# fallenshock/SinDDM

Hardware: AMD Instinct MI355X
Metric: diffusion steps/sec (finest scale) + imgs/sec full multi-scale sample, 1/2/4/8 GPU (higher is better)
Workload: dtype f32 (3x3 convs: binary16 hi/lo split products -- Winograd-domain GEMMs with all 4 MFMA terms, fp32 accumulate; fp32-equivalent, error vs float64 = the fp32 oracle's: tests/test_gpu_h2.py; everything else fp32); 1 GPU; C3: 6-scale pyramid, T=1000, finest scale 411x512, batch 64 per GPU, dim=160; batch_per_gpu=64, global_batch=64, scale=5, parallelism=independent chains over 1 GPU(s), one all-gather of the images

## Files before the change

### sinddm_amd/csrc/conv_args.h

```cpp
#pragma once
#include "common.h"

namespace sinddm {

struct ConvArgs {
    const float* in;
    const float* in2;
    const float* resid;
    const float* aux;
    const float* w3;
    const float* w1;
    const float* bias;
    const float* zero;
    float* out;
    float* out_pre;
    int B, H, W, Cin, Cin2, Cout;
    int nch3, nch1;
    int tilesX, tilesY, ntiles, tiles_per_xcd;
    int coblks;
    int mtp;
    int act;
    const float* wsinv;
    const float* amax_in;
    float* amax_out;
    int Wt;
};

template <int NT, int WV = 4>
struct ConvGeom {
    static constexpr int TW = 32;
    static constexpr int TPR = TW / 16;
    static constexpr int RPW = NT / TPR;
    static constexpr int TH = WV * RPW;
    static constexpr int RS = TW + 2;
    static constexpr int HR = TH + 2;
    static constexpr int PS = ((HR * RS - 16 + 31) / 32) * 32 + 16;
    static constexpr int IN_ELEMS = KC * HR * RS;
    static constexpr int IREGS = (IN_ELEMS + CONV_THREADS - 1) / CONV_THREADS;
};

template <int MT, int NT, int WV = 4>
struct ConvCfg {
    using G = ConvGeom<NT, WV>;
    static constexpr int CO_LDS = (MT * 16) % 32 == 16 ? MT * 16 : MT * 16 + 16;
    static constexpr int W3_F4 = 9 * KC * CO_LDS / 4;
    static constexpr int W1_F4 = KC * CO_LDS / 4;
    static constexpr int WREGS = (W3_F4 + CONV_THREADS - 1) / CONV_THREADS;
    static constexpr int LDS_FLOATS = 9 * KC * CO_LDS + KC * G::PS;
};

struct ConvProfiler {
    bool on = false;
    int used = 0;
    double flops = 0.0;
    double exec_flops = 0.0;
    static constexpr int MAXREC = 8192;
    hipEvent_t ev[2 * MAXREC];
    int created = 0;
    unsigned char kind[MAXREC];
    unsigned char gen[MAXREC];
    double rec_flops[MAXREC], rec_exec[MAXREC];
    void note(int k, double fl, double ex, int g = 0) {
        kind[used] = (unsigned char)k; gen[used] = (unsigned char)g; rec_flops[used] = fl; rec_exec[used] = ex;
        flops += fl; exec_flops += ex; ++used;
    }
    bool begin(hipStream_t st) {
        if (!on || used >= MAXREC) return false;
        while (created <= used) {
            (void)hipEventCreate(&ev[2 * created]);
            (void)hipEventCreate(&ev[2 * created + 1]);
            ++created;
        }
        (void)hipEventRecord(ev[2 * used], st);
        return true;
    }
    void end(hipStream_t st, int k, double fl, double ex, int g = 0) {
        (void)hipEventRecord(ev[2 * used + 1], st);
        note(k, fl, ex, g);
    }
};
ConvProfiler& conv_profiler();

}
```

### sinddm_amd/csrc/conv_wh.h

```cpp
#pragma once
#include <utility>
#include "split16.h"

namespace sinddm {

template <class F, int... I>
__device__ __forceinline__ void wh_static_for_impl(F&& f, std::integer_sequence<int, I...>) {
    (f(std::integral_constant<int, I>{}), ...);
}
template <int N, class F>
__device__ __forceinline__ void wh_static_for(F&& f) {
    wh_static_for_impl(f, std::make_integer_sequence<int, N>{});
}

#ifndef WH_ABL
#define WH_ABL 0
#endif
#ifndef WH_MIXLO
#define WH_MIXLO 1
#endif
#ifndef WH_NT
#define WH_NT 6
#endif
#ifdef WH_TIMING
__device__ unsigned long long g_wh_seg[8 * 256 * 8 * 32];
#define WH_SEG(slot) do { if (j == 2) g_wh_seg[((p.mtp * 256 + blockIdx.x) * 8 + wv) * 32 + (slot)] = __builtin_amdgcn_s_memtime(); } while (0)
#else
#define WH_SEG(slot) do {} while (0)
#endif
constexpr int WH_TH = 8, WH_TW = 32;
constexpr int WH_RS = 40;
constexpr int WH_PS = 408;
constexpr int WH_RAW = 16 * WH_PS * 4;
constexpr int WH_V = 24 * 2 * 64 * 16;
constexpr int WH_XS = 36;
constexpr int WH_X = 2 * 6 * 32 * WH_XS * 4;
constexpr int WH_LDS = 160 * 1024;
constexpr int WH_REGION = WH_LDS - WH_RAW;
constexpr int WH_VB = WH_REGION - WH_V;
static_assert(WH_X <= WH_VB && WH_V + WH_X <= WH_REGION && WH_VB % 16 == 0, "exchange buffer beside either V buffer");
constexpr int WH_TARGET_EXP = 10;
constexpr int WH_COB = 80;

inline bool wh_shape_ok(int cin, int cout) { return cin >= 32 && cin % 16 == 0 && cout % WH_COB == 0; }
inline long long wh_image_halfs(int cin, int cout) { return (long long)(cout / WH_COB) * (cin / 16) * 24 * 5 * 512; }

__device__ __forceinline__ int wh_shift_for(float m, int target) {
    const unsigned bits = __float_as_uint(m) & 0x7fffffffu;
    const int e = (int)(bits >> 23);
    if (e == 0 || e == 255) return 0;
    int s = target - (e - 127);
    return s > 100 ? 100 : (s < -100 ? -100 : s);
}

__device__ __forceinline__ void wh_u24(const float* __restrict__ w, long long base, int transpose, double (&u)[24]) {
    const double G2[4][3] = {{1., 0., 0.}, {.5, .5, .5}, {.5, -.5, .5}, {0., 0., 1.}};
    const double G4[6][3] = {{1. / 4, 0., 0.}, {-1. / 6, -1. / 6, -1. / 6}, {-1. / 6, 1. / 6, -1. / 6},
                             {1. / 24, 1. / 12, 1. / 6}, {1. / 24, -1. / 12, 1. / 6}, {0., 0., 1.}};
    double g[3][3];
#pragma unroll
    for (int a = 0; a < 3; ++a)
#pragma unroll
        for (int b = 0; b < 3; ++b) g[a][b] = (double)(transpose ? w[base + (2 - a) * 3 + (2 - b)] : w[base + a * 3 + b]);
#pragma unroll
    for (int i = 0; i < 4; ++i)
#pragma unroll
        for (int j = 0; j < 6; ++j) {
            double acc = 0.;
#pragma unroll
            for (int a = 0; a < 3; ++a) {
                double r = 0.;
#pragma unroll
                for (int b = 0; b < 3; ++b) r += G4[j][b] * g[a][b];
                acc += G2[i][a] * r;
            }
            u[i * 6 + j] = acc;
        }
}

__global__ __launch_bounds__(256) void wh_wscale_kernel(const float* __restrict__ w, float* __restrict__ wsinv, int cin,
                                                         int cout, int transpose) {
    const int m = blockIdx.x;
    const int M = transpose ? cin : cout, K = transpose ? cout : cin;
    float mx = 0.f;
    if (m < M)
        for (int k = threadIdx.x; k < K; k += 256) {
            double u[24];
            wh_u24(w, transpose ? ((long long)k * cin + m) * 9 : ((long long)m * cin + k) * 9, transpose, u);
#pragma unroll
            for (int f = 0; f < 24; ++f) mx = fmaxf(mx, fabsf((float)u[f]));
        }
    __shared__ float red[4];
#pragma unroll
    for (int o = 32; o > 0; o >>= 1) mx = fmaxf(mx, __shfl_xor(mx, o));
    if ((threadIdx.x & 63) == 0) red[threadIdx.x >> 6] = mx;
    __syncthreads();
    if (threadIdx.x == 0 && m < M) {
        mx = fmaxf(fmaxf(red[0], red[1]), fmaxf(red[2], red[3]));
        wsinv[m] = h2_pow2(-h2_shift_for(mx));
    }
}

__global__ __launch_bounds__(256) void wh_pack_kernel(const float* __restrict__ w, const float* __restrict__ wsinv,
                                                       _Float16* __restrict__ img, int cin, int cout, int transpose,
                                                       long long total) {
    const long long i = (long long)blockIdx.x * 256 + threadIdx.x;
    if (i >= total) return;
    const int M = transpose ? cin : cout, K = transpose ? cout : cin;
    const int nch = K / 16;
    long long r = i;
    const int e = (int)(r % 8); r /= 8;
    const int co16 = (int)(r % 16); r /= 16;
    const int kh = (int)(r % 2); r /= 2;
    const int n = (int)(r % 5); r /= 5;
    const int ch = (int)(r % nch); r /= nch;
    const int cb = (int)r;
    const int m = cb * WH_COB + n * 16 + co16;
    const int k = ch * 16 + kh * 8 + e;
    double u[24];
    if (m < M && k < K) wh_u24(w, transpose ? ((long long)k * cin + m) * 9 : ((long long)m * cin + k) * 9, transpose, u);
    else {
#pragma unroll
        for (int f = 0; f < 24; ++f) u[f] = 0.;
    }
    const double sc = m < M ? 1.0 / (double)wsinv[m] : 1.0;
#pragma unroll
    for (int f = 0; f < 24; ++f) {
        const double s = u[f] * sc;
        const _Float16 hi = (_Float16)(float)s;
        const _Float16 lo = (_Float16)(float)(s - (double)(float)hi);
        const long long o = ((((long long)(cb * nch + ch) * 24 + f) * 5 + n) * 2) * 256 + (kh * 16 + co16) * 8 + e;
        img[o] = hi;
        img[o + 256] = lo;
    }
}

inline int wh_pack_launch(const float* w, float* wsinv, void* img, int cin, int cout, int transpose, hipStream_t st) {
    const int M = transpose ? cin : cout, K = transpose ? cout : cin;
    hipLaunchKernelGGL(wh_wscale_kernel, dim3(M), dim3(256), 0, st, w, wsinv, cin, cout, transpose);
    SINDDM_LAUNCH_CHECK();
    const long long total = (long long)(M / WH_COB) * (K / 16) * 5 * 2 * 16 * 8;
    hipLaunchKernelGGL(wh_pack_kernel, dim3((unsigned)((total + 255) / 256)), dim3(256), 0, st, w, wsinv,
                       static_cast<_Float16*>(img), cin, cout, transpose, total);
    SINDDM_LAUNCH_CHECK();
    return 0;
}

__device__ __forceinline__ void wh_barrier() { asm volatile("s_waitcnt lgkmcnt(0)\n\ts_barrier" ::: "memory"); }

__device__ __forceinline__ float wh_dpp_shr2(float old, float src) {
    return __builtin_bit_cast(float, __builtin_amdgcn_update_dpp(__builtin_bit_cast(int, old), __builtin_bit_cast(int, src), 0x112, 0xf, 0xf, false));
}
__device__ __forceinline__ float wh_dpp_shl2(float old, float src) {
    return __builtin_bit_cast(float, __builtin_amdgcn_update_dpp(__builtin_bit_cast(int, old), __builtin_bit_cast(int, src), 0x102, 0xf, 0xf, false));
}

__global__ __launch_bounds__(512) void conv_wh_kernel(ConvArgs p, int items_per_xcd, int wg_per_xcd) {
    typedef __attribute__((address_space(3))) float lds_f;
    extern __shared__ __attribute__((aligned(16))) float smem[];
    unsigned char* const sbytes = reinterpret_cast<unsigned char*>(smem);
    unsigned char* const sRaw = sbytes;
    unsigned char* const sV = sbytes + WH_RAW;
    const unsigned lds0 = (unsigned)(size_t)(lds_f*)smem;

    const int tid = threadIdx.x;
    const int lane = tid & 63;
    const int wv = __builtin_amdgcn_readfirstlane(tid >> 6);
    const int l16 = lane & 15, kq = lane >> 4;
    const int H = p.H, W = p.W;
    const int HW = H * W;
    const int Wt = p.Wt > 0 ? p.Wt : W;
    const int nch = p.nch3;
    const bool big_out = __builtin_amdgcn_readfirstlane((size_t)p.B * p.Cout * HW > ((size_t)1 << 28)) != 0;
    constexpr int OOB = 0x40000000;
    const bool service_rt = wv >= 6;
    const int sv = wv - 6;

    const int t_q = lane & 1, t_tc = (lane >> 1) & 7, t_mg = (lane >> 4) & 1, t_trl = lane >> 5;
    const int t_tr = t_mg * 2 + t_trl, t_t16 = t_trl * 8 + t_tc;
    const int t_rdB = (((sv & 1) * 8 + 4 * t_q) * WH_PS + 2 * t_tr * WH_RS + 4 * t_tc + 4) * 4;
    const int t_rdE = (((sv & 1) * 8 + 4 * t_q) * WH_PS + 2 * t_tr * WH_RS + (t_tc == 7 ? 36 : 3)) * 4;
    const int t_wr0 = ((t_mg * 64 + (sv & 1) * 16 + t_t16) * 16) + t_q * 8;
    const int fj = service_rt ? 0 : wv;
    const int a_rd = ((kq & 1) * 16 + l16) * 16;

    const int xcd = blockIdx.x & 7, ls = blockIdx.x >> 3;
    const int tpi = p.tilesX * p.tilesY;
    struct Item { int b, y0, x0, cb; bool ok; };
    auto decode = [&](int j) {
        Item it;
        const int li = ls + j * wg_per_xcd;
        const int tl = li / p.coblks;
        it.cb = li - tl * p.coblks;
        const int tile = xcd * p.tiles_per_xcd + tl;
        it.ok = li < items_per_xcd && tile < p.ntiles;
        const int tcl = it.ok ? tile : 0;
        it.b = tcl / tpi;
        const int trm = tcl - it.b * tpi;
        const int tyi = trm / p.tilesX;
        it.y0 = tyi * WH_TH;
        it.x0 = (trm - tyi * p.tilesX) * WH_TW;
        return it;
    };
    auto stage_offsets = [&](const Item& it, int (&vo)[2]) {
#pragma unroll
        for (int ps = 0; ps < 2; ++ps) {
            const int qd = ps * 64 + lane;
            const int r = qd / 10, g = qd - r * 10;
            const int gy = it.y0 - 1 + r, gx = it.x0 - 4 + 4 * g;
            vo[ps] = (qd < 100 && gy >= 0 && gy < H && gx >= 0 && gx < W) ? (gy * W + gx) * 4 : OOB;
        }
    };
    auto role_body = [&](auto ROLE) {
    constexpr bool service = decltype(ROLE)::value;
    f32x4 stg[16];
    auto stage_load = [&](const __amdgpu_buffer_rsrc_t& rs, const int (&vo)[2], int c) {
#pragma unroll
        for (int k = 0; k < 8; ++k) {
            const int so = (c * 16 + (sv & 1) * 8 + k) * HW * 4;
            stg[2 * k] = (WH_ABL & 1) ? f32x4{0.f, 0.f, 0.f, 0.f} : __builtin_bit_cast(f32x4, __builtin_amdgcn_raw_buffer_load_b128(rs, vo[0], so, (WH_NT & 1) ? 2 : 0));
            stg[2 * k + 1] = (WH_ABL & 1) ? f32x4{0.f, 0.f, 0.f, 0.f} : __builtin_bit_cast(f32x4, __builtin_amdgcn_raw_buffer_load_b128(rs, vo[1], so, (WH_NT & 1) ? 2 : 0));
        }
    };
    auto stage_write = [&](unsigned char* raw) {
        unsigned char* dst = raw + (sv & 1) * 8 * WH_PS * 4 + lane * 16;
#pragma unroll
        for (int k = 0; k < 8; ++k) {
            *reinterpret_cast<f32x4*>(dst + k * WH_PS * 4) = stg[2 * k];
            if (lane < 36) *reinterpret_cast<f32x4*>(dst + k * WH_PS * 4 + 1024) = stg[2 * k + 1];
        }
    };
    auto in_rsrc = [&](int b) {
        return __builtin_amdgcn_make_buffer_rsrc(const_cast<float*>(p.in + (size_t)b * p.Cin * HW), 0, p.Cin * HW * 4, 0x00020000);
    };

    Item cur = decode(0);
    if (!cur.ok) return;
    int svoff[2] = {OOB, OOB};
#ifndef WH_SVC_PRIO
#define WH_SVC_PRIO 2
#endif
    if constexpr (service) __builtin_amdgcn_s_setprio(WH_SVC_PRIO);
    if constexpr (service) {
        stage_offsets(cur, svoff);
        stage_load(in_rsrc(cur.b), svoff, 0);
    }
    auto item_scale = [&](const Item& it, float& sxo, float& inv) {
        const int xs = p.amax_in ? wh_shift_for(p.amax_in[(size_t)it.b * AMAX_STRIDE], WH_TARGET_EXP) : 0;
        const float sg = (((it.x0 >> 5) + (it.y0 >> 3) + it.b) & 1) ? -1.0f : 1.0f;
        sxo = sg * h2_pow2(xs);
        inv = sg * h2_pow2(-xs);
    };
    int g = 0;
    auto vbuf = [&](int k) { return sV + ((k & 1) ? WH_VB : 0); };
    for (int j = 0;; ++j) {
        const Item nxt = decode(j + 1);
        const int cb = cur.cb, b = cur.b, y0 = cur.y0, x0 = cur.x0;
        float sx, inv_sx;
        item_scale(cur, sx, inv_sx);

        const __amdgpu_buffer_rsrc_t rsin = in_rsrc(b);

        auto transform = [&](const unsigned char* raw, unsigned char* vb, float sxv) {
            if (WH_ABL & 2) return;
            const f32x2 sx2{sxv, sxv};
            const unsigned char* rpB = raw + t_rdB;
            const unsigned char* rpE = raw + t_rdE;
            unsigned char* wp = vb + t_wr0;
            f32x2 d[2][4][6];
#pragma unroll
            for (int pr = 0; pr < 2; ++pr)
#pragma unroll
                for (int rr = 0; rr < 4; ++rr) {
                    const int o = ((2 * pr) * WH_PS + rr * WH_RS) * 4;
                    const f32x4 a4 = *reinterpret_cast<const f32x4*>(rpB + o), b4 = *reinterpret_cast<const f32x4*>(rpB + o + WH_PS * 4);
                    const float ae = *reinterpret_cast<const float*>(rpE + o), be = *reinterpret_cast<const float*>(rpE + o + WH_PS * 4);
                    d[pr][rr][0] = f32x2{wh_dpp_shr2(ae, a4[3]), wh_dpp_shr2(be, b4[3])};
                    d[pr][rr][1] = f32x2{a4[0], b4[0]}; d[pr][rr][2] = f32x2{a4[1], b4[1]};
                    d[pr][rr][3] = f32x2{a4[2], b4[2]}; d[pr][rr][4] = f32x2{a4[3], b4[3]};
                    d[pr][rr][5] = f32x2{wh_dpp_shl2(ae, a4[0]), wh_dpp_shl2(be, b4[0])};
                }
            wh_static_for<4>([&](auto II) {
                constexpr int i = decltype(II)::value;
                h16x2 hi[2][6], lo[2][6];
#pragma unroll
                for (int pr = 0; pr < 2; ++pr) {
                    f32x2 r[6];
#pragma unroll
                    for (int c = 0; c < 6; ++c)
                        r[c] = i == 0 ? d[pr][0][c] - d[pr][2][c] : i == 1 ? d[pr][1][c] + d[pr][2][c]
                             : i == 2 ? d[pr][2][c] - d[pr][1][c] : d[pr][1][c] - d[pr][3][c];
                    const f32x2 s24 = r[4] - 4.f * r[2], s13 = r[3] - 4.f * r[1];
                    const f32x2 u24 = r[4] - r[2], d31 = r[3] - r[1];
                    f32x2 v[6];
                    v[0] = 4.f * r[0] + (r[4] - 5.f * r[2]);
                    v[1] = s24 + s13;
                    v[2] = s24 - s13;
                    v[3] = u24 + 2.f * d31;
                    v[4] = u24 - 2.f * d31;
                    v[5] = 4.f * r[1] + (r[5] - 5.f * r[3]);
#pragma unroll
                    for (int j = 0; j < 6; ++j) {
                        const f32x2 sc = v[j] * sx2;
                        hi[pr][j] = __builtin_convertvector(sc, h16x2);
#if WH_MIXLO
                        lo[pr][j] = h16x2{(_Float16)__builtin_fmaf(v[j].x, sxv, -(float)hi[pr][j].x), (_Float16)__builtin_fmaf(v[j].y, sxv, -(float)hi[pr][j].y)};
#else
                        const f32x2 rem{__builtin_fmaf(v[j].x, sxv, -(float)hi[pr][j].x), __builtin_fmaf(v[j].y, sxv, -(float)hi[pr][j].y)};
                        lo[pr][j] = __builtin_convertvector(rem, h16x2);
#endif
                    }
                }
#pragma unroll
                for (int j = 0; j < 6; ++j) {
                    using h16x4 = __attribute__((ext_vector_type(4))) _Float16;
                    *reinterpret_cast<h16x4*>(wp + (i * 6 + j) * 2048) = h16x4{hi[0][j][0], hi[0][j][1], hi[1][j][0], hi[1][j][1]};
                    *reinterpret_cast<h16x4*>(wp + (i * 6 + j) * 2048 + 512) = h16x4{lo[0][j][0], lo[0][j][1], lo[1][j][0], lo[1][j][1]};
                }
            });
        };

        f32x4 acc[4][2][5];
#pragma unroll
        for (int a = 0; a < 4; ++a)
#pragma unroll
            for (int g = 0; g < 2; ++g)
#pragma unroll
                for (int n = 0; n < 5; ++n) acc[a][g][n] = f32x4{0.f, 0.f, 0.f, 0.f};
        const __amdgpu_buffer_rsrc_t rsw =
            __builtin_amdgcn_make_buffer_rsrc(const_cast<float*>(p.w3), 0, 0x7FFFFFF0, 0x00020000);
        const int wlane = lane * 16;
        const int wbase = ((cb * nch) * 24 + fj) * 5 * 1024;
        h16x8 ur[10];
        auto load_u = [&](int c, int fi, int n, int slot) {
            const int so = wbase + (c * 24 * 5 + fi * 30 + n) * 1024;
            ur[slot] = __builtin_bit_cast(h16x8, __builtin_amdgcn_raw_buffer_load_b128(rsw, wlane, so, 0));
        };
        auto multiply = [&](int c, const unsigned char* vb) {
            const unsigned char* A = vb + fj * 2048 + a_rd;
            wh_static_for<4>([&](auto FI) {
                constexpr int fi = decltype(FI)::value;
                constexpr int fo = fi * 6 * 2048;
                h16x8 ah0, ah1, al0, al1;
                ah0 = *reinterpret_cast<const h16x8*>(A + fo);
                ah1 = *reinterpret_cast<const h16x8*>(A + fo + 1024);
                al0 = *reinterpret_cast<const h16x8*>(A + fo + 512);
                al1 = *reinterpret_cast<const h16x8*>(A + fo + 1024 + 512);
                wh_static_for<5>([&](auto NN) {
                    constexpr int n = decltype(NN)::value;
                    constexpr int slot = (fi & 1) * 5 + n;
                    const h16x8 u = ur[slot];
                    __builtin_amdgcn_sched_barrier(0);
                    if (WH_ABL & 8) {
                        asm volatile("" ::"v"(ah0), "v"(ah1), "v"(al0), "v"(al1), "v"(u));
                    } else {
                        acc[fi][0][n] = __builtin_amdgcn_mfma_f32_16x16x32_f16(al0, u, acc[fi][0][n], 0, 0, 0);
                        acc[fi][1][n] = __builtin_amdgcn_mfma_f32_16x16x32_f16(al1, u, acc[fi][1][n], 0, 0, 0);
                        acc[fi][0][n] = __builtin_amdgcn_mfma_f32_16x16x32_f16(ah0, u, acc[fi][0][n], 0, 0, 0);
                        acc[fi][1][n] = __builtin_amdgcn_mfma_f32_16x16x32_f16(ah1, u, acc[fi][1][n], 0, 0, 0);
                    }
                    __builtin_amdgcn_sched_barrier(0);
                    if (!(WH_ABL & 4)) {
                        if (fi < 2) load_u(c, fi + 2, n, slot);
                        else load_u(c + 1 < nch ? c + 1 : c, fi - 2, n, slot);
                    }
                    __builtin_amdgcn_sched_barrier(0);
                });
            });
        };

        const int e_t = tid & 31, e_co = tid >> 5;
        const int e_tr = e_t >> 3, e_tc = e_t & 7;
        const int ey = y0 + 2 * e_tr, ex = x0 + 4 * e_tc;
        f32x4 rsd[5][2];
        float ek[5], ebv[5];
        auto ep_operands = [&]() {
            const bool e_in = ex < W;
#pragma unroll
            for (int n = 0; n < 5; ++n) {
                const int co = cb * WH_COB + n * 16 + e_co;
                ek[n] = inv_sx * p.wsinv[co];
                ebv[n] = p.bias ? p.bias[co] : 0.0f;
#pragma unroll
                for (int pp = 0; pp < 2; ++pp) {
                    rsd[n][pp] = f32x4{0.f, 0.f, 0.f, 0.f};
                    if (p.resid && !(WH_ABL & 16) && e_in && ey + pp < H)
                        rsd[n][pp] = ((WH_NT & 2) && big_out) ? __builtin_nontemporal_load(reinterpret_cast<const f32x4*>(p.resid + ((size_t)b * p.Cout + co) * HW + (size_t)(ey + pp) * W + ex))
                                                 : *reinterpret_cast<const f32x4*>(p.resid + ((size_t)b * p.Cout + co) * HW + (size_t)(ey + pp) * W + ex);
                }
            }
        };

        WH_SEG(0);
        if constexpr (service) {
            const __amdgpu_buffer_rsrc_t rsnx = in_rsrc(nxt.ok ? nxt.b : b);
            float sxn = 0.f, inv_n = 0.f;
            if (nxt.ok) item_scale(nxt, sxn, inv_n);
            if (j == 0) {
                stage_write(sRaw);
                if (nch > 1) stage_load(rsin, svoff, 1);
                else if (nxt.ok) { stage_offsets(nxt, svoff); stage_load(rsnx, svoff, 0); }
                WH_SEG(1);
                transform(sRaw, vbuf(g), sx);
                wh_barrier();
            }
            WH_SEG(2);
            for (int c = 0; c < nch; ++c) {
                if (c + 1 < nch || nxt.ok) {
                    stage_write(sRaw);
                    if (c + 2 < nch) stage_load(rsin, svoff, c + 2);
                    else if (nxt.ok) {
                        if (c + 2 == nch) stage_offsets(nxt, svoff);
                        if (c + 2 == nch || nch > 1) stage_load(rsnx, svoff, c + 2 - nch);
                    }
                    if (c == 3) WH_SEG(24);
                    transform(sRaw, vbuf(g + c + 1), c + 1 < nch ? sx : sxn);
                    if (c == 3) WH_SEG(25);
                }
                wh_barrier();
                if (c < 12) WH_SEG(3 + c);
            }
            ep_operands();
        } else {
            wh_static_for<10>([&](auto SL) {
                constexpr int sl = decltype(SL)::value;
                load_u(0, sl / 5, sl % 5, sl);
            });
            WH_SEG(1);
            if (j == 0) wh_barrier();
            WH_SEG(2);
            for (int c = 0; c < nch; ++c) {
                multiply(c, vbuf(g + c));
                if (c == 3) WH_SEG(25);
                wh_barrier();
                if (c < 12) WH_SEG(3 + c);
            }
            ep_operands();
        }
        g += nch;
        WH_SEG(16);

        const int e_wr = ((fj * 32 + l16) * WH_XS + 4 * kq) * 4;
        const int e_rd = (e_co * WH_XS + e_t) * 4;
        float amax = 0.f;
        WH_SEG(17);
        if constexpr (!service) {
#pragma unroll
            for (int mg = 0; mg < 2; ++mg)
#pragma unroll
                for (int n = 0; n < 5; ++n) {
                    acc[0][mg][n] = acc[0][mg][n] + acc[1][mg][n] + acc[2][mg][n];
                    acc[1][mg][n] = acc[1][mg][n] - acc[2][mg][n] - acc[3][mg][n];
                }
        }
        wh_static_for<3>([&](auto PS) {
            constexpr int n0 = 2 * decltype(PS)::value;
            constexpr int nn = n0 + 2 <= 5 ? 2 : 1;
            unsigned char* X = sV + ((g & 1) ? 0 : WH_V);
            if constexpr (!service) {
#pragma unroll
                for (int r = 0; r < 2; ++r)
#pragma unroll
                    for (int nl = 0; nl < nn; ++nl)
#pragma unroll
                        for (int mg = 0; mg < 2; ++mg)
                            *reinterpret_cast<f32x4*>(X + e_wr + (r * 6 * 32 + nl * 16) * (WH_XS * 4) + mg * 64) = acc[r][mg][n0 + nl];
            }
            wh_barrier();
            WH_SEG(18 + decltype(PS)::value);
            float q[nn][2][6];
#pragma unroll
            for (int nl = 0; nl < nn; ++nl)
#pragma unroll
                for (int r = 0; r < 2; ++r)
#pragma unroll
                    for (int j = 0; j < 6; ++j)
                        q[nl][r][j] = *reinterpret_cast<const float*>(X + e_rd + ((r * 6 + j) * 32 + nl * 16) * (WH_XS * 4));
            wh_barrier();
            wh_static_for<nn>([&](auto NL) {
                constexpr int n = n0 + decltype(NL)::value;
                const int co = cb * WH_COB + n * 16 + e_co;
                const float k = ek[n];
                const float bv = ebv[n];
#pragma unroll
                for (int pp = 0; pp < 2; ++pp) {
                    const float* z = q[decltype(NL)::value][pp];
                    const float s12 = z[1] + z[2], d12 = z[1] - z[2], s34 = z[3] + z[4], d34 = z[3] - z[4];
                    f32x4 v{z[0] + s12 + s34, d12 + 2.f * d34, s12 + 4.f * s34, d12 + 8.f * d34 + z[5]};
                    const int y = ey + pp;
                    if ((WH_ABL & 16) && v[0] != 123.456f) continue;
                    if (y < H && ex < W) {
                        const size_t o = ((size_t)b * p.Cout + co) * HW + (size_t)y * W + ex;
                        v = v * k + bv;
                        if (p.out_pre) *reinterpret_cast<f32x4*>(p.out_pre + o) = v;
                        if (p.act == 1) v = gelu_erf4(v);
                        else if (p.act == 2) {
                            const f32x4 a = *reinterpret_cast<const f32x4*>(p.aux + o);
#pragma unroll
                            for (int e = 0; e < 4; ++e) v[e] *= gelu_erf_grad(a[e]);
                        }
                        v += rsd[n][pp];
                        if (ex + 4 > Wt) {
#pragma unroll
                            for (int e = 0; e < 4; ++e) v[e] = ex + e < Wt ? v[e] : 0.0f;
                        }
#pragma unroll
                        for (int e = 0; e < 4; ++e) amax = fmaxf(amax, fabsf(v[e]));
                        if ((WH_NT & 4) && big_out) __builtin_nontemporal_store(v, reinterpret_cast<f32x4*>(p.out + o));
                        else *reinterpret_cast<f32x4*>(p.out + o) = v;
                    }
                }
            });
        });
        if (p.amax_out) amax_publish(amax, p.amax_out + (size_t)b * AMAX_STRIDE);
        WH_SEG(23);
        if (!nxt.ok) break;
        cur = nxt;
    }
    };
    if (service_rt) role_body(std::true_type{});
    else role_body(std::false_type{});
}

#ifndef SINDDM_WH_MIN_ITEMS_PER_CU
#define SINDDM_WH_MIN_ITEMS_PER_CU 12
#endif
#ifndef SINDDM_WH_MIN_PIXELS
#define SINDDM_WH_MIN_PIXELS 12000
#endif
#ifndef SINDDM_CONV_WH
#define SINDDM_CONV_WH 1
#endif
inline bool conv_wh_applies(bool fp32_convs, int B, int H, int W, int cin, int cout) {
    if (!SINDDM_CONV_WH || fp32_convs || !wh_shape_ok(cin, cout) || W % 4 != 0) return false;
    if ((long long)cin * H * W * 4 >= 0x40000000LL) return false;
    if ((long long)H * W < SINDDM_WH_MIN_PIXELS) return false;
    return (long long)B * ((W + WH_TW - 1) / WH_TW) * ((H + WH_TH - 1) / WH_TH) * (cout / WH_COB) >=
           (long long)SINDDM_WH_MIN_ITEMS_PER_CU * cu_count();
}

inline int conv_wh_launch(const ConvArgs& a_in, hipStream_t st) {
    ConvArgs a = a_in;
    if (!wh_shape_ok(a.Cin, a.Cout) || a.W % 4 != 0 || !a.wsinv || (long long)a.Cin * a.H * a.W * 4 >= 0x40000000LL)
        return SINDDM_E_BADSHAPE;
    ConvProfiler& prof = conv_profiler();
    const bool rec = prof.begin(st);
    a.nch3 = a.Cin / 16;
    a.coblks = a.Cout / WH_COB;
    a.tilesX = (a.W + WH_TW - 1) / WH_TW;
    a.tilesY = (a.H + WH_TH - 1) / WH_TH;
    a.ntiles = a.B * a.tilesX * a.tilesY;
    a.tiles_per_xcd = (a.ntiles + 7) / 8;
    const int ipx = a.tiles_per_xcd * a.coblks;
    int wpx = cu_count() / 8;
    if (wpx < 1) wpx = 1;
    if (wpx > ipx) wpx = ipx;
    static const hipError_t attr_rc = hipFuncSetAttribute(reinterpret_cast<const void*>(&conv_wh_kernel),
                                                          hipFuncAttributeMaxDynamicSharedMemorySize, WH_LDS);
    if (attr_rc != hipSuccess) return (int)attr_rc;
#ifdef WH_TIMING
    static int wh_launch_no = 0;
    a.mtp = wh_launch_no++ % 8;
#endif
    hipLaunchKernelGGL(conv_wh_kernel, dim3(wpx * 8), dim3(512), WH_LDS, st, a, ipx, wpx);
    if (rec) {
        const double fl = 2.0 * a.B * a.H * (a.Wt > 0 ? a.Wt : a.W) * (double)a.Cout * 9.0 * a.Cin;
        prof.end(st, 1, fl, 2.0 * a.ntiles * 32.0 * 24.0 * 4.0 * (double)a.Cout * a.Cin, 8);
    }
    SINDDM_LAUNCH_CHECK();
    return 0;
}

}
```

Baseline: 780.3 sample-steps/s (finest scale, batch x steps/s, all GPUs).

## Prefetch residual via buffer loads overlapped with last-channel MFMA loop

During the final input-channel iteration of the Winograd conv, the weight prefetch registers are reused to issue buffer loads of the residual tensor. The next-channel weight loads are redirected to a zero-sized resource so they return nothing. Residual values are thus fetched while the last GEMMs run, instead of being loaded serially in the epilogue, hiding global-memory latency. The change adds a resid_buf flag, a restructured loop exit so the epilogue loads happen before the final barrier, and a fallback path when the residual is too large for a buffer offset.

New measurement: 781.0 sample-steps/s (finest scale, batch x steps/s, all GPUs) (median of 4 runs). No clear change (+0.1%).

```diff
diff --git a/sinddm_amd/csrc/conv_args.h b/sinddm_amd/csrc/conv_args.h
--- a/sinddm_amd/csrc/conv_args.h
+++ b/sinddm_amd/csrc/conv_args.h
@@ -24,6 +24,7 @@
     const float* amax_in;
     float* amax_out;
     int Wt;
+    int resid_buf;
 };
 
 template <int NT, int WV = 4>
diff --git a/sinddm_amd/csrc/conv_wh.h b/sinddm_amd/csrc/conv_wh.h
--- a/sinddm_amd/csrc/conv_wh.h
+++ b/sinddm_amd/csrc/conv_wh.h
@@ -173,6 +173,7 @@
     const int nch = p.nch3;
     const bool big_out = __builtin_amdgcn_readfirstlane((size_t)p.B * p.Cout * HW > ((size_t)1 << 28)) != 0;
     constexpr int OOB = 0x40000000;
+    constexpr int ROOB = (int)0x80000000u;
     const bool service_rt = wv >= 6;
     const int sv = wv - 6;
 
@@ -320,6 +321,20 @@
             });
         };
 
+        const int e_t = tid & 31, e_co = tid >> 5;
+        const int e_tr = e_t >> 3, e_tc = e_t & 7;
+        const int ey = y0 + 2 * e_tr, ex = x0 + 4 * e_tc;
+        const __amdgpu_buffer_rsrc_t rsr = __builtin_amdgcn_make_buffer_rsrc(
+            const_cast<float*>(p.resid + (size_t)b * p.Cout * HW), 0, (p.resid_buf && !(WH_ABL & 16)) ? p.Cout * HW * 4 : 0, 0x00020000);
+        int rvo[2];
+#pragma unroll
+        for (int pp = 0; pp < 2; ++pp) rvo[pp] = (ex < W && ey + pp < H) ? ((e_co * H + ey + pp) * W + ex) * 4 : ROOB;
+        const int rso = cb * WH_COB * HW * 4;
+        auto load_resid = [&](int n, int pp) {
+            if ((WH_NT & 2) && big_out) return __builtin_bit_cast(f32x4, __builtin_amdgcn_raw_buffer_load_b128(rsr, rvo[pp], rso + n * 16 * HW * 4, 2));
+            return __builtin_bit_cast(f32x4, __builtin_amdgcn_raw_buffer_load_b128(rsr, rvo[pp], rso + n * 16 * HW * 4, 0));
+        };
+
         f32x4 acc[4][2][5];
 #pragma unroll
         for (int a = 0; a < 4; ++a)
@@ -329,6 +344,7 @@
                 for (int n = 0; n < 5; ++n) acc[a][g][n] = f32x4{0.f, 0.f, 0.f, 0.f};
         const __amdgpu_buffer_rsrc_t rsw =
             __builtin_amdgcn_make_buffer_rsrc(const_cast<float*>(p.w3), 0, 0x7FFFFFF0, 0x00020000);
+        const __amdgpu_buffer_rsrc_t rsw0 = __builtin_amdgcn_make_buffer_rsrc(const_cast<float*>(p.w3), 0, 0, 0x00020000);
         const int wlane = lane * 16;
         const int wbase = ((cb * nch) * 24 + fj) * 5 * 1024;
         h16x8 ur[10];
@@ -338,6 +354,15 @@
         };
         auto multiply = [&](int c, const unsigned char* vb) {
             const unsigned char* A = vb + fj * 2048 + a_rd;
+            const bool last = c + 1 == nch;
+            const __amdgpu_buffer_rsrc_t rs2 = last ? rsw0 : rsw;
+            auto resid_request = [&](auto S0) {
+                if (!last || !p.resid_buf) return;
+                wh_static_for<5>([&](auto SL) {
+                    constexpr int sl = decltype(S0)::value + decltype(SL)::value;
+                    ur[sl] = __builtin_bit_cast(h16x8, load_resid(sl >> 1, sl & 1));
+                });
+            };
             wh_static_for<4>([&](auto FI) {
                 constexpr int fi = decltype(FI)::value;
                 constexpr int fo = fi * 6 * 2048;
@@ -362,25 +387,29 @@
                     __builtin_amdgcn_sched_barrier(0);
                     if (!(WH_ABL & 4)) {
                         if (fi < 2) load_u(c, fi + 2, n, slot);
-                        else load_u(c + 1 < nch ? c + 1 : c, fi - 2, n, slot);
+                        else ur[slot] = __builtin_bit_cast(h16x8, __builtin_amdgcn_raw_buffer_load_b128(rs2, wlane, wbase + ((c + 1) * 24 * 5 + (fi - 2) * 30 + n) * 1024, 0));
                     }
                     __builtin_amdgcn_sched_barrier(0);
                 });
+                if constexpr (fi >= 2) resid_request(std::integral_constant<int, (fi & 1) * 5>{});
             });
         };
 
-        const int e_t = tid & 31, e_co = tid >> 5;
-        const int e_tr = e_t >> 3, e_tc = e_t & 7;
-        const int ey = y0 + 2 * e_tr, ex = x0 + 4 * e_tc;
         f32x4 rsd[5][2];
         float ek[5], ebv[5];
-        auto ep_operands = [&]() {
-            const bool e_in = ex < W;
+        auto ep_scales = [&]() {
 #pragma unroll
             for (int n = 0; n < 5; ++n) {
                 const int co = cb * WH_COB + n * 16 + e_co;
                 ek[n] = inv_sx * p.wsinv[co];
                 ebv[n] = p.bias ? p.bias[co] : 0.0f;
+            }
+        };
+        auto ep_resid_late = [&]() {
+            const bool e_in = ex < W;
+#pragma unroll
+            for (int n = 0; n < 5; ++n) {
+                const int co = cb * WH_COB + n * 16 + e_co;
 #pragma unroll
                 for (int pp = 0; pp < 2; ++pp) {
                     rsd[n][pp] = f32x4{0.f, 0.f, 0.f, 0.f};
@@ -405,7 +434,7 @@
                 wh_barrier();
             }
             WH_SEG(2);
-            for (int c = 0; c < nch; ++c) {
+            for (int c = 0;; ++c) {
                 if (c + 1 < nch || nxt.ok) {
                     stage_write(sRaw);
                     if (c + 2 < nch) stage_load(rsin, svoff, c + 2);
@@ -417,10 +446,19 @@
                     transform(sRaw, vbuf(g + c + 1), c + 1 < nch ? sx : sxn);
                     if (c == 3) WH_SEG(25);
                 }
+                if (c + 1 == nch) break;
                 wh_barrier();
                 if (c < 12) WH_SEG(3 + c);
             }
-            ep_operands();
+            ep_scales();
+            if (p.resid_buf) {
+#pragma unroll
+                for (int n = 0; n < 5; ++n)
+#pragma unroll
+                    for (int pp = 0; pp < 2; ++pp) rsd[n][pp] = load_resid(n, pp);
+            } else ep_resid_late();
+            wh_barrier();
+            if (nch <= 12) WH_SEG(2 + nch);
         } else {
             wh_static_for<10>([&](auto SL) {
                 constexpr int sl = decltype(SL)::value;
@@ -429,13 +467,23 @@
             WH_SEG(1);
             if (j == 0) wh_barrier();
             WH_SEG(2);
-            for (int c = 0; c < nch; ++c) {
+#pragma nounroll
+            for (int c = 0;; ++c) {
                 multiply(c, vbuf(g + c));
                 if (c == 3) WH_SEG(25);
+                if (c + 1 == nch) break;
                 wh_barrier();
                 if (c < 12) WH_SEG(3 + c);
             }
-            ep_operands();
+            ep_scales();
+            if (p.resid_buf) {
+#pragma unroll
+                for (int n = 0; n < 5; ++n)
+#pragma unroll
+                    for (int pp = 0; pp < 2; ++pp) rsd[n][pp] = __builtin_bit_cast(f32x4, ur[2 * n + pp]);
+            } else ep_resid_late();
+            wh_barrier();
+            if (nch <= 12) WH_SEG(2 + nch);
         }
         g += nch;
         WH_SEG(16);
@@ -551,6 +599,7 @@
     a.tilesY = (a.H + WH_TH - 1) / WH_TH;
     a.ntiles = a.B * a.tilesX * a.tilesY;
     a.tiles_per_xcd = (a.ntiles + 7) / 8;
+    a.resid_buf = a.resid && (long long)a.Cout * a.H * a.W * 4 < 0x80000000LL;
     const int ipx = a.tiles_per_xcd * a.coblks;
     int wpx = cu_count() / 8;
     if (wpx < 1) wpx = 1;
```
